# waldstein94/Stratified-Transformer

Measured on AMD Instinct MI355X. Metric: points/sec through StratifiedAttention fwd+bwd, 100k-pt scene, higher is better.
Workload: dtype f32

## Files before the change

include/pointops2_hip.h:

```cpp
#ifndef POINTOPS2_HIP_H
#define POINTOPS2_HIP_H

#include <stddef.h>
#include <stdint.h>

#ifdef __cplusplus
extern "C" {
#endif

void pointops2_set_stream(void *hip_stream);
void *pointops2_get_stream(void);
const char *pointops2_last_error(void);
int pointops2_abi_version(void);
void pointops2_diag_set_fps_patience(unsigned long long ticks_100mhz);


void furthestsampling_cuda_launcher(int b, int n, const float *xyz, const int *offset,
                                    const int *new_offset, float *tmp, int *idx);

void knnquery_cuda_launcher(int m, int nsample, const float *xyz, const float *new_xyz,
                            const int *offset, const int *new_offset, int *idx, float *dist2);

void grouping_forward_cuda_launcher(int m, int nsample, int c, const float *input, const int *idx, float *output);
void grouping_backward_cuda_launcher(int m, int nsample, int c, const float *grad_output, const int *idx, float *grad_input);
// ... 164 lines not shown
size_t pointops2_cell_plan_workspace_bytes(int N);
void pointops2_cell_plan_count_launcher(int N, int max_queries, const int *s_cluster, const int *s_starts, const int *l_cluster,
                                        const int *ls_starts, int *cell_order, int *qcell, int *cell_desc, int *cell_qstart,
                                        int *cell_kbase, int *cell_pbase, int *cell_perm, int *parent_first, int *counts, void *ws,
                                        size_t ws_bytes);
void pointops2_cell_plan_prepare_launcher(int N, int max_queries, const int *s_cluster, const int *l_cluster, int *cell_order,
                                          int *parent_first, int *counts, void *ws, size_t ws_bytes);
void pointops2_cell_plan_sizes_launcher(int N, const int *s_cluster, const int *s_starts, const int *l_cluster, const int *ls_starts,
                                        const int *cell_order, int *qcell, int *cell_desc, int *cell_qstart, int *cell_kbase,
                                        int *cell_pbase, int *cell_perm, int *counts, void *ws, size_t ws_bytes);
void pointops2_cell_plan_fill_launcher(int N, const float *xyz, float window, float quant, int L, const int *s_order, const int *ls,
                                       const float *wc, const int *cell_order, const int *qcell, const int *cell_qstart,
                                       const int *cell_desc, const int *cell_kbase, const int *cell_pbase, int *cell_keys, int *kcell,
                                       unsigned int *relp);
void pointops2_swin_quant_launcher(int N, const float *xyz, const float *bbox6, float window, float quant, int shifted, int *q);
void pointops2_swin_pairs_rel_launcher(int N, int M, const int *index_0, const int *index_1, const int *q, int qgl, int *rel_idx);
void pointops2_swin_cell_fill_launcher(int N, int L, int qgl, const int *q, const int *s_order, const int *ls, const float *wc,
                                       const int *cell_order, const int *qcell, const int *cell_qstart, const int *cell_desc,
                                       const int *cell_kbase, const int *cell_pbase, int *cell_keys, int *kcell, unsigned int *relp);
void cell_attention_forward_launcher(const pointops2_cell_plan *plan, int h, int hdim, int L, const float *q, const float *k,
                                     const float *v, const float *table_q, const float *table_k, const float *table_v, float *out,
                                     float *ml, float *pbuf);
void cell_attention_backward_launcher(const pointops2_cell_plan *plan, int h, int hdim, int L, const float *grad_out, const float *q,
                                      const float *k, const float *v, const float *out, const float *table_q, const float *table_k,
                                      const float *table_v, const float *pbuf, float *gsbuf, float *grad_q, float *grad_k,
                                      float *grad_v, float *grad_table_q, float *grad_table_k, float *grad_table_v);
#define POINTOPS2_CELL_FWD_ERROR   (-1)
#define POINTOPS2_CELL_FWD_NONE    0
#define POINTOPS2_CELL_FWD_MFMA64  1
#define POINTOPS2_CELL_FWD_MFMA80  2
#define POINTOPS2_CELL_FWD_VALU80  3
#define POINTOPS2_CELL_FWD_VALU160 4
int pointops2_cell_forward_variant(const pointops2_cell_plan *plan, int h, int hdim, int L, int bf16);

void pointops2_voxel_keys_launcher(int N, int is_f64, const void *coord, double voxel, unsigned long long *keys);
void pointops2_crop_dist_launcher(int N, int is_f64, const void *coord, int seed, void *dist);

void cell_attention_forward_bf16_launcher(const pointops2_cell_plan *plan, int h, int hdim, int L, const uint16_t *q, const uint16_t *k,
                                          const uint16_t *v, const uint16_t *table_q, const uint16_t *table_k, const uint16_t *table_v,
                                          float *out, float *ml, float *pbuf);
void cell_attention_backward_bf16_launcher(const pointops2_cell_plan *plan, int h, int hdim, int L, const float *grad_out, const uint16_t *q,
                                           const uint16_t *k, const uint16_t *v, const float *out, const uint16_t *table_q,
                                           const uint16_t *table_k, const uint16_t *table_v, const float *pbuf, float *gsbuf, float *grad_q,
                                           float *grad_k, float *grad_v, float *grad_table_q, float *grad_table_k, float *grad_table_v);
#define POINTOPS2_ROWS_F32  0
#define POINTOPS2_ROWS_F16  1
#define POINTOPS2_ROWS_BF16 2
void cell_attention_qkv_forward_launcher(const pointops2_cell_plan *plan, int h, int hdim, int L, const void *qkv, int row_type, float scale,
                                         const float *table_q, const float *table_k, const float *table_v, float *out, float *ml, float *pbuf);
void cell_attention_qkv_backward_launcher(const pointops2_cell_plan *plan, int h, int hdim, int L, const float *grad_out, const void *qkv, int row_type,
                                          float scale, const float *out, const float *table_q, const float *table_k, const float *table_v,
                                          const float *pbuf, float *gsbuf, float *grad_qkv, float *grad_table_q, float *grad_table_k,
                                          float *grad_table_v);

void kpconv_aggregate_forward_launcher(int n_q, int n_s, int n_nb, int c, int n_kp, const float *query_xyz, const float *support_xyz,
                                       const int *neighbors, const float *feat, const float *k_points, float extent, float *wf);
void kpconv_aggregate_backward_launcher(int n_q, int n_s, int n_nb, int c, int n_kp, const float *query_xyz, const float *support_xyz,
                                        const int *neighbors, const float *k_points, float extent, const float *grad_wf,
                                        float *grad_feat);

void grouped_max_forward_launcher(int m, int n_s, int k, int c, int row_type, const void *feat, const int *idx, void *out,
                                  unsigned char *arg);
void grouped_max_backward_launcher(int m, int n_s, int k, int c, int row_type, const void *grad_out, const unsigned char *arg,
                                   const int *src_offsets, const int *src_pair, void *grad_feat);

void residual_norm_forward_launcher(int n, int c, int y_type, int o_type, const float *x, const void *y, const float *s, const float *gamma,
// ... 124 lines not shown
```

stratified_transformer_amd/_lib.py:

```python
import ctypes
import os
import subprocess

import torch

_HERE = os.path.dirname(os.path.abspath(__file__))
LIB_PATH = os.path.join(_HERE, "lib", "libpointops2_hip.so")
CSRC = os.path.join(_HERE, "csrc")
_lib = None

I, U, P, Z, F, D = ctypes.c_int, ctypes.c_uint, ctypes.c_void_p, ctypes.c_size_t, ctypes.c_float, ctypes.c_double
Q = ctypes.c_longlong


class LaunchOpts(ctypes.Structure):
    _fields_ = [("table_rows", I), ("key_rows", I), ("csc_offsets", P), ("csc_pair", P), ("csc_query", P), ("row_order", P),
                ("row_order_rows", I), ("workspace", P), ("workspace_bytes", Z), ("point_count", I), ("batch_count", I),
                ("fps_prev_idx", P), ("fps_prev_new_offset", P), ("fps_unordered", I)]


def with_table_rows(opts, L):
    opts = opts if opts is not None else LaunchOpts()
    opts.table_rows = int(L)
    return opts
# ... 80 lines not shown
    "pointops2_dbscan_core_launcher": [I, I, P, P, P, P, P, P, P, P],
    "pointops2_dbscan_round_launcher": [I, I, P, P, P, P, P, P, P],
    "pointops2_dbscan_label_launcher": [I, I, P, P, P, P, P, P, P, P],
    "pointops2_contacts_count_launcher": [I, I, P, P, P, F, P, P],
    "pointops2_contacts_min_launcher": [I, I, P, P],
    "pointops2_label_boxes_launcher": [I, I, P, P, P, P, P],
    "pointops2_reach_rows_launcher": [I, I, P, P, P, F, P],
    "pointops2_supports_keys_launcher": [I, I, P, P, P, D, I, I, I, P],
    "pointops2_supports_means_launcher": [I, I, I, P, P, P, P, P, P, P, P],
    "pointops2_supports_count_launcher": [I, P, P, F, I, P],
    "pointops2_evaltile_seed_dist_launcher": [I, I, P, P, P, P, P, P],
    "pointops2_evaltile_update_launcher": [I, I, I, P, P, P, P, P],
    "pointops2_evaltile_vote_launcher": [I, I, I, I, P, P, P, P, P],
    "pointops2_evaltile_vote_shift_launcher": [I, I, I, I, P, I, P, P, P, P, P, P],
    "pointops2_augment_pass_launcher": [I] * 6 + [P] * 10,
    "pointops2_augment_blur_launcher": [Q, I, I, P, P, P],
    "optim_adamw_step_launcher": [I, I, P, P, Z, P, P, I],
    "optim_step_launcher": [I, I, I, P, P, Z, P, P, I, D, P],
    "residual_norm_stream_forward_launcher": [I, I, I, I, I, P, P, P, P, P, F, P, P, P],
    "residual_norm_stream_backward_launcher": [I, I, I, I, I, P, P, P, P, P, P, P, P, P, I, P, P],
}
RESULTS = {
    "pointops2_get_stream": ([], P),
    "pointops2_last_error": ([], ctypes.c_char_p),
    "pointops2_abi_version": ([], I),
    "pointops2_csc_workspace_bytes": ([I, I], Z),
    "pointops2_fps_workspace_bytes": ([I, I], Z),
    "pointops2_knn_workspace_bytes": ([I, I, I], Z),
    "pointops2_index_workspace_bytes": ([I], Z),
    "pointops2_partitions4_workspace_bytes": ([I], Z),
    "pointops2_row_order_workspace_bytes": ([I], Z),
    "pointops2_cell_plan_workspace_bytes": ([I], Z),
    "pointops2_cell_forward_variant": ([P, I, I, I, I], I),
    "pointops2_evaltile_max_parts": ([], I),
    "pointops2_optim_workspace_bytes": ([I, I], Z),
    "pointops2_optim_step_workspace_bytes": ([I, I, Q], Z),
}
OPTIM_KINDS = {"adamw": 0, "sgd": 1}

CELL_FWD = {"error": -1, "none": 0, "mfma64": 1, "mfma80": 2, "valu80": 3, "valu160": 4}
ROW_TYPES = {torch.float32: 0, torch.float16: 1, torch.bfloat16: 2}
ACTIVATIONS = {"none": 0, "relu": 1, "leaky_relu": 2, "tanh": 3}


def cell_forward_variant(plan, h, L, bf16=False, hdim=16):
    arg = None if plan is None else plan.c_arg() if hasattr(plan, "c_arg") else ctypes.byref(plan)
    code = lib().pointops2_cell_forward_variant(arg, int(h), int(hdim), int(L), int(bool(bf16)))
    return {v: k for k, v in CELL_FWD.items()}[code]


def exported_symbols():
    return sorted(list(SIGNATURES) + list(RESULTS))


def build(verbose=False):
    cmd = ["make", "-C", CSRC, "-j8"] + ([] if verbose else ["-s"])
    subprocess.check_call(cmd)
    return LIB_PATH


def lib():
    global _lib
    if _lib is None:
        if not os.path.exists(LIB_PATH):
            raise RuntimeError(
                f"{LIB_PATH} is missing: the HIP extension has not been built "
                "(run `python -c 'import __graft_entry__ as g; g.build()'` or `make -C stratified_transformer_amd/csrc`). "
                "There is no CPU fallback for the product path.")
        l = ctypes.CDLL(LIB_PATH)
        for name, argtypes in SIGNATURES.items():
            fn = getattr(l, name)
            fn.argtypes = argtypes
            fn.restype = None
        for name, (argtypes, restype) in RESULTS.items():
            fn = getattr(l, name)
            fn.argtypes = argtypes
            fn.restype = restype
        _lib = l
    return _lib


# ... 37 lines not shown
```

stratified_transformer_amd/csrc/cell_attn.hip:

```cpp
#include "cell_common.h"

namespace p2 {


template <typename T>
__device__ __forceinline__ void stage_table_t(T *lds, const T *__restrict__ tab, int L, int h, int head) {
    const int total = 3 * L * 16;
    for (int x = threadIdx.x; x < total; x += blockDim.x) {
        const int i = x % 16, r = (x / 16) % L, ax = x / (16 * L);
        lds[x] = tab[(((size_t)r * h + head) * 16 + i) * 3 + ax];
    }
}
template <int TS, typename T>
__device__ __forceinline__ void stage_tables(T *lds, const T *__restrict__ table_q, const T *__restrict__ table_k, const T *__restrict__ table_v, int L,
                                             int h, int head) {
    stage_table_t<T>(lds, table_q, L, h, head);
    stage_table_t<T>(lds + TS, table_k, L, h, head);
    stage_table_t<T>(lds + 2 * TS, table_v, L, h, head);
    __syncthreads();
}

template <int LCAP>
struct TabGeo {
    static constexpr int TS = 3 * LCAP * 16;
// ... 68 lines not shown
    __device__ __forceinline__ float4 q_row4(const RT *q, int i) const {
        if constexpr (PK) return scaled_row4<RT>(q + (size_t)i * rs_packed + hoff, qscale);
        else return ld_row4(q + (size_t)i * C + hoff);
    }
};
template <typename TT, bool PK>
__device__ __forceinline__ LaneCtx<TT, PK> make_lane_ctx(const TT *lds, int h, int L, int rs, float qscale) {
    LaneCtx<TT, PK> x;
    x.lds = lds;
    x.L = L;
    x.h = h;
    x.head = blockIdx.y;
    x.C = h * 16;
    x.rs_packed = rs;
    x.qscale = qscale;
    x.lane = threadIdx.x & 63;
    x.p = x.lane >> 2;
    x.c = x.lane & 3;
    x.hoff = x.head * 16 + 4 * x.c;
    return x;
}

__device__ __forceinline__ void wait_vmem() {
    asm volatile("" ::: "memory");
    __builtin_amdgcn_s_waitcnt(0x0F70);
}
__device__ __forceinline__ int next_query_ids(rsrc_t qid, int off) {
    const int ids = (int)bload_u32(qid, off);
    wait_vmem();
    return ids;
}

template <int NPA, typename RT, typename T, bool PK>
__device__ __forceinline__ void load_key_rows(const LaneCtx<T, PK> &x, const CellBufs &cb, const RT *__restrict__ rows, int j0, int nvalid,
                                              float4 (&r4)[NPA]) {
    unsigned keys[NPA];
    bload_words<NPA>(cb.key, (j0 + x.p * NPA) * 4, keys);
#pragma unroll
    for (int t = 0; t < NPA; t++) {
        const float4 r = ld_row4(rows + (size_t)keys[t] * x.rs() + x.hoff);
        r4[t] = t < nvalid ? r : make_float4(0.f, 0.f, 0.f, 0.f);
    }
}

template <int NPA, int TS, typename RT, typename T, bool PK>
__device__ __forceinline__ void fwd_sweep_logits(const LaneCtx<T, PK> &x, const CellTask &ct, const CellBufs &cb, rsrc_t rs_p,
                                                 const RT *__restrict__ q, const RT *__restrict__ k, float *__restrict__ ml,
                                                 int ch, bool single, int j0, int nkc) {
    const int p = x.p, c = x.c;
    const int nvalid = min(max(nkc - p * NPA, 0), NPA);
    float4 k4[NPA];
    load_key_rows<NPA, RT, T, PK>(x, cb, k, j0, nvalid, k4);
    int ids = (int)bload_u32(cb.qid, x.lane * 4);
    int i_nx = __builtin_amdgcn_readlane(ids, 0);
    float4 q4_nx = x.q_row4(q, i_nx);
    unsigned w_nx[NPA];
    bload_words<NPA>(cb.rel, (j0 + p * NPA) * 4, w_nx);
    float lg_pv[NPA];
#pragma unroll
    for (int t = 0; t < NPA; t++) lg_pv[t] = 0.f;
#pragma unroll 1
    for (int il = 0; il < ct.nq; il++) {
        wait_vmem();
        const int i = i_nx;
        const float4 q4 = q4_nx;
        unsigned w[NPA];
#pragma unroll
        for (int t = 0; t < NPA; t++) w[t] = w_nx[t];
        const int roff = (il * ct.nk + j0 + p * NPA) * 4;
        if (((il + 1) & 63) == 0) ids = next_query_ids(cb.qid, (il + 1 + x.lane) * 4);
        i_nx = __builtin_amdgcn_readlane(ids, (il + 1) & 63);
        q4_nx = x.q_row4(q, i_nx);
        bload_words<NPA>(cb.rel, roff + ct.nk * 4, w_nx);
        if (single && il && c == 0) bstore_floats<NPA>(rs_p, roff - ct.nk * 4, lg_pv, nvalid);
        float lg[NPA];
// ... 111 lines not shown
                                                                 const T *__restrict__ table_v, float *__restrict__ out,
                                                                 float *__restrict__ ml, float *__restrict__ pbuf, size_t plane) {
    constexpr int TS = TabGeo<LCAP>::TS;
    extern __shared__ float lds_raw[];
    T *lds = reinterpret_cast<T *>(lds_raw);
    const LaneCtx<T, PK> x = make_lane_ctx<T, PK>(lds, h, L, rs, qscale);
    const int wave = __builtin_amdgcn_readfirstlane(threadIdx.x >> 6);
    stage_tables<TS, T>(lds, table_q, table_k, table_v, L, h, x.head);
    const int nC = share_count(pl, pl.counts[0]);
    float *pb = pbuf + (size_t)x.head * plane;
    const int slots = gridDim.x * CA_WAVES, slot = blockIdx.x * CA_WAVES + wave;
    for (int round = 0; round * slots < nC; round++) {
        const int task = snake_task(round, slot, slots);
        if (task >= nC) continue;
        const CellTask ct = cell_task(pl, share_task(pl, task));
        const int nch = (ct.nk + 16 * NP - 1) / (16 * NP);
        const CellBufs cb = make_cell_bufs(pl, ct);
        const rsrc_t rs_p = tile_rsrc(pb, ct);
        for (int ch = 0; ch < nch; ch++) {
            const int j0 = ch * 16 * NP, nkc = min(16 * NP, ct.nk - j0);
            dispatch_passes<NP>((nkc + 15) >> 4, [&](auto tag) {
                fwd_sweep_logits<decltype(tag)::value, TS, RT, T, PK>(x, ct, cb, rs_p, q, k, ml, ch, nch == 1, j0, nkc);
            });
        }
        for (int ch = 0; ch < nch; ch++) {
            const int j0 = ch * 16 * NP, nkc = min(16 * NP, ct.nk - j0);
            dispatch_passes<NP>((nkc + 15) >> 4, [&](auto tag) {
                fwd_sweep_values<decltype(tag)::value, TS, RT, T, PK>(x, ct, cb, rs_p, v, ml, out, ch, nch == 1, j0, nkc);
            });
        }
    }
}

template <int NPA, typename T, bool PK>
__device__ __forceinline__ void flush_key_grads(float *scr, const float4 (&acc)[NPA], rsrc_t rs_key, int j0, int nkc, float *__restrict__ grad,
                                                const LaneCtx<T, PK> &x) {
    unsigned keys[4][NPA];
#pragma unroll
    for (int kk = 0; kk < 4; kk++) bload_words<NPA>(rs_key, (j0 + ((x.lane >> 4) + 4 * kk) * NPA) * 4, keys[kk]);
    wait_vmem();
#pragma unroll
    for (int t = 0; t < NPA; t++) {
        *reinterpret_cast<float4 *>(scr + x.p * 16 + 4 * x.c) = acc[t];
        __builtin_amdgcn_s_waitcnt(0xC07F);
        __builtin_amdgcn_wave_barrier();
#pragma unroll
        for (int kk = 0; kk < 4; kk++) {
            const int s = (x.lane >> 4) + 4 * kk;
            if (s * NPA + t < nkc) unsafeAtomicAdd(grad + (size_t)keys[kk][t] * x.rs() + x.head * 16 + (x.lane & 15), scr[s * 16 + (x.lane & 15)]);
        }
        __builtin_amdgcn_s_waitcnt(0xC07F);
        __builtin_amdgcn_wave_barrier();
    }
}

template <int NPA, int TS, typename RT, typename T, bool PK>
__device__ __forceinline__ void bwd_sweep_values(const LaneCtx<T, PK> &x, const CellTask &ct, const CellBufs &cb, rsrc_t rs_p, rsrc_t rs_g,
                                                 float *scr, const float *__restrict__ go, const float *__restrict__ out,
                                                 const RT *__restrict__ v, float *__restrict__ grad_v, int j0, int nkc) {
    const int p = x.p, c = x.c;
    const int nvalid = min(max(nkc - p * NPA, 0), NPA);
    float4 v4[NPA], dv4[NPA];
    load_key_rows<NPA, RT, T, PK>(x, cb, v, j0, nvalid, v4);
#pragma unroll
    for (int t = 0; t < NPA; t++) dv4[t] = make_float4(0.f, 0.f, 0.f, 0.f);
    unsigned w_nx[NPA];
    float a_nx[NPA];
    bload_words<NPA>(cb.rel, (j0 + p * NPA) * 4, w_nx);
    bload_floats<NPA>(rs_p, (j0 + p * NPA) * 4, a_nx);
    int ids = (int)bload_u32(cb.qid, x.lane * 4);
    int i_nx = __builtin_amdgcn_readlane(ids, 0);
    float4 go_nx = ldg4(go + (size_t)i_nx * x.C + x.hoff), o_nx = ldg4(out + (size_t)i_nx * x.C + x.hoff);
    float gs_pv[NPA];
#pragma unroll
    for (int t = 0; t < NPA; t++) gs_pv[t] = 0.f;
#pragma unroll 1
    for (int il = 0; il < ct.nq; il++) {
        wait_vmem();
        const int roff = (il * ct.nk + j0 + p * NPA) * 4;
        const float4 go4 = go_nx, o4 = o_nx;
        unsigned w[NPA];
        float a[NPA];
#pragma unroll
        for (int t = 0; t < NPA; t++) {
            w[t] = w_nx[t];
            a[t] = t < nvalid ? a_nx[t] : 0.f;
        }
        if (((il + 1) & 63) == 0) ids = next_query_ids(cb.qid, (il + 1 + x.lane) * 4);
        i_nx = __builtin_amdgcn_readlane(ids, (il + 1) & 63);
        go_nx = ldg4(go + (size_t)i_nx * x.C + x.hoff);
        o_nx = ldg4(out + (size_t)i_nx * x.C + x.hoff);
        bload_words<NPA>(cb.rel, roff + ct.nk * 4, w_nx);
        bload_floats<NPA>(rs_p, roff + ct.nk * 4, a_nx);
        if (il && c == 0) bstore_floats<NPA>(rs_g, roff - ct.nk * 4, gs_pv, nvalid);
        const float delta = quad_sum(pdot4(go4, o4));
        Rows3 rv = rows_at<2 * TS, T>(x.lds, row_off(w[0], x.L, c));
#pragma unroll
        for (int t = 0; t < NPA; t++) {
            Rows3 rv1 = rv;
            if (t + 1 < NPA) rv1 = rows_at<2 * TS, T>(x.lds, row_off(w[t + 1], x.L, c));
            const float ga = quad_sum(pdot4(go4, padd4(rsum(rv), v4[t])));
            gs_pv[t] = a[t] * (ga - delta);
            dv4[t] = pfma4(a[t], go4, dv4[t]);
            rv = rv1;
            __builtin_amdgcn_sched_barrier(0);
        }
    }
    if (ct.nq > 0 && c == 0) bstore_floats<NPA>(rs_g, ((ct.nq - 1) * ct.nk + j0 + p * NPA) * 4, gs_pv, nvalid);
    flush_key_grads<NPA, T, PK>(scr, dv4, cb.key, j0, nkc, grad_v, x);
}

template <int NPA, int TS, typename RT, typename T, bool PK>
__device__ __forceinline__ void bwd_sweep_keys(const LaneCtx<T, PK> &x, const CellTask &ct, const CellBufs &cb, rsrc_t rs_g, float *scr,
                                               const RT *__restrict__ q, const RT *__restrict__ k, float *__restrict__ grad_q,
                                               float *__restrict__ grad_k, int ch, int j0, int nkc) {
    const int p = x.p, c = x.c;
    const int nvalid = min(max(nkc - p * NPA, 0), NPA);
    float4 k4[NPA], dk4[NPA];
    load_key_rows<NPA, RT, T, PK>(x, cb, k, j0, nvalid, k4);
#pragma unroll
    for (int t = 0; t < NPA; t++) dk4[t] = make_float4(0.f, 0.f, 0.f, 0.f);
    unsigned w_nx[NPA];
    float g_nx[NPA];
    bload_words<NPA>(cb.rel, (j0 + p * NPA) * 4, w_nx);
    bload_floats<NPA>(rs_g, (j0 + p * NPA) * 4, g_nx);
    int ids = (int)bload_u32(cb.qid, x.lane * 4);
    int i_nx = __builtin_amdgcn_readlane(ids, 0);
    float4 q_nx = x.q_row4(q, i_nx);
    float4 tot_pv = make_float4(0.f, 0.f, 0.f, 0.f);
    int i_pv = 0;
    auto store_dq = [&](int i, float4 tot) {
        float *o = grad_q + (size_t)i * x.rs() + x.hoff;
        stg4(o, ch ? add4(tot, ldg4(o)) : tot);
    };
#pragma unroll 1
    for (int il = 0; il < ct.nq; il++) {
        wait_vmem();
        const int i = i_nx;
        const int roff = (il * ct.nk + j0 + p * NPA) * 4;
        const float4 q4 = q_nx;
        unsigned w[NPA];
        float g[NPA];
#pragma unroll
        for (int t = 0; t < NPA; t++) {
            w[t] = w_nx[t];
            g[t] = t < nvalid ? g_nx[t] : 0.f;
        }
        if (((il + 1) & 63) == 0) ids = next_query_ids(cb.qid, (il + 1 + x.lane) * 4);
        i_nx = __builtin_amdgcn_readlane(ids, (il + 1) & 63);
        q_nx = x.q_row4(q, i_nx);
        bload_words<NPA>(cb.rel, roff + ct.nk * 4, w_nx);
        bload_floats<NPA>(rs_g, roff + ct.nk * 4, g_nx);
        if (il && p == 0) store_dq(i_pv, tot_pv);
        float4 dq = make_float4(0.f, 0.f, 0.f, 0.f);
        RowOff ro = row_off(w[0], x.L, c);
        Rows3 rq = rows_at<0, T>(x.lds, ro), rk = rows_at<TS, T>(x.lds, ro);
#pragma unroll
        for (int t = 0; t < NPA; t++) {
            Rows3 rq1 = rq, rk1 = rk;
            if (t + 1 < NPA) {
                ro = row_off(w[t + 1], x.L, c);
                rq1 = rows_at<0, T>(x.lds, ro);
                rk1 = rows_at<TS, T>(x.lds, ro);
            }
            dq = pfma4(g[t], padd4(rsum(rq), k4[t]), dq);
            dk4[t] = pfma4(g[t], padd4(rsum(rk), q4), dk4[t]);
            rq = rq1;
            rk = rk1;
            __builtin_amdgcn_sched_barrier(0);
        }
        float4 tot = slots_sum16_4(dq);
        if constexpr (PK) tot = make_float4(tot.x * x.qscale, tot.y * x.qscale, tot.z * x.qscale, tot.w * x.qscale);
        tot_pv = tot;
        i_pv = i;
    }
    if (ct.nq > 0 && p == 0) store_dq(i_pv, tot_pv);
    flush_key_grads<NPA, T, PK>(scr, dk4, cb.key, j0, nkc, grad_k, x);
}

template <int NP, int LCAP, typename RT, typename T, bool PK>
__global__ __launch_bounds__(CA_WAVES_BWD * 64) void cell_bwd_kernel(pointops2_cell_plan pl, int h, int L, const float *__restrict__ go,
                                                                 const RT *__restrict__ q, const RT *__restrict__ k,
                                                                 const RT *__restrict__ v, int rs, float qscale, const float *__restrict__ out,
                                                                 const T *__restrict__ table_q, const T *__restrict__ table_k,
                                                                 const T *__restrict__ table_v, const float *__restrict__ pbuf,
                                                                 float *__restrict__ gsbuf, size_t plane, float *__restrict__ grad_q,
                                                                 float *__restrict__ grad_k, float *__restrict__ grad_v) {
    constexpr int TS = TabGeo<LCAP>::TS;
    extern __shared__ float lds_raw[];
    T *lds = reinterpret_cast<T *>(lds_raw);
    const LaneCtx<T, PK> x = make_lane_ctx<T, PK>(lds, h, L, rs, qscale);
    const int wave = __builtin_amdgcn_readfirstlane(threadIdx.x >> 6);
    float *scr = reinterpret_cast<float *>(lds + 3 * TS) + wave * 256;
    stage_tables<TS, T>(lds, table_q, table_k, table_v, L, h, x.head);
    const int nC = share_count(pl, pl.counts[0]);
    const float *pb = pbuf + (size_t)x.head * plane;
    float *gb = gsbuf + (size_t)x.head * plane;
    const int slots = gridDim.x * CA_WAVES_BWD, slot = blockIdx.x * CA_WAVES_BWD + wave;
    for (int round = 0; round * slots < nC; round++) {
        const int task = snake_task(round, slot, slots);
        if (task >= nC) continue;
        const CellTask ct = cell_task(pl, share_task(pl, task));
        const int nch = (ct.nk + 16 * NP - 1) / (16 * NP);
        const CellBufs cb = make_cell_bufs(pl, ct);
        const rsrc_t rs_p = tile_rsrc(pb, ct), rs_g = tile_rsrc(gb, ct);
        for (int ch = 0; ch < nch; ch++) {
            const int j0 = ch * 16 * NP, nkc = min(16 * NP, ct.nk - j0);
            dispatch_passes<NP>((nkc + 15) >> 4, [&](auto tag) {
                bwd_sweep_values<decltype(tag)::value, TS, RT, T, PK>(x, ct, cb, rs_p, rs_g, scr, go, out, v, grad_v, j0, nkc);
            });
        }
        for (int ch = 0; ch < nch; ch++) {
            const int j0 = ch * 16 * NP, nkc = min(16 * NP, ct.nk - j0);
            dispatch_passes<NP>((nkc + 15) >> 4, [&](auto tag) {
                bwd_sweep_keys<decltype(tag)::value, TS, RT, T, PK>(x, ct, cb, rs_g, scr, q, k, grad_q, grad_k, ch, j0, nkc);
            });
        }
    }
}

struct CFixScale {
    float mul, inv;
};
__device__ __forceinline__ CFixScale c_row_scale(unsigned maxbits, int n) {
    CFixScale sc;
    if (maxbits >= 0x7f800000u) {
        sc.mul = 0.f;
        sc.inv = __uint_as_float(0x7fc00000u);
        return sc;
    }
    const int E = (int)(maxbits >> 23) - 126;
    const int bits_n = 32 - __clz(max(n, 1));
    const int S = max(-126, min(126, 30 - bits_n - E));
    sc.mul = __uint_as_float((unsigned)(S + 127) << 23);
    sc.inv = __uint_as_float((unsigned)(127 - S) << 23);
    return sc;
}

constexpr int CT_WAVES = 8;

template <int TA>
struct CellTableGeo {
    static constexpr int LP = TA * 16;
    static constexpr int ROW = 3 * LP + 16;
    static constexpr size_t walk_bytes() { return (size_t)CT_WAVES * 4 * ROW * 4; }
    static constexpr size_t sum_bytes() { return (size_t)LP * 48 * 4; }
    static constexpr size_t lds_bytes() { return walk_bytes() > sum_bytes() ? walk_bytes() : sum_bytes(); }
};
// ... 177 lines not shown
static void launch_valu_fwd(hipStream_t st, const pointops2_cell_plan *plan, int h, int L, const CellRows<RT> &r, const CellTables<TT> &t, float *out, float *ml,
                            float *pbuf) {
    const size_t lds = TabGeo<LCAP>::bytes(sizeof(TT));
    allow_big_lds(cell_fwd_kernel<CA_NP, LCAP, RT, TT, PK>, lds);
    const dim3 grid(cell_grid_x(1, plan->n_cells, h, CA_WAVES), h);
    hipLaunchKernelGGL((cell_fwd_kernel<CA_NP, LCAP, RT, TT, PK>), grid, dim3(CA_WAVES * 64), lds, st, *plan, h, L, r.q, r.k, r.v, r.rs, r.scale, t.q, t.k, t.v, out,
                       ml, pbuf, (size_t)plan->n_pairs);
}

template <typename RT, typename TT, bool PK>
static void launch_cell_fwd(hipStream_t st, const pointops2_cell_plan *plan, int h, int hdim, int L, const CellRows<RT> &r, const CellTables<TT> &t, float *out,
                            float *ml, float *pbuf) {
    const char *why;
    const int variant = cell_fwd_variant(plan, h, hdim, L, !std::is_same<TT, float>::value, &why);
    if (why != nullptr) { set_error(why); return; }
    if (variant == POINTOPS2_CELL_FWD_NONE) return;
    if constexpr (std::is_same<TT, float>::value) {
        if (variant == POINTOPS2_CELL_FWD_MFMA64 || variant == POINTOPS2_CELL_FWD_MFMA80) {
            cell_fwd_mfma_launch(st, variant, plan, h, L, RowTag<RT>::code, PK, CellRows<void>{r.q, r.k, r.v, r.rs, r.scale}, t, out, pbuf);
            check_launch();
            return;
        }
    }
    if (variant == POINTOPS2_CELL_FWD_VALU80) launch_valu_fwd<80, RT, TT, PK>(st, plan, h, L, r, t, out, ml, pbuf);
    else launch_valu_fwd<160, RT, TT, PK>(st, plan, h, L, r, t, out, ml, pbuf);
    check_launch();
}

template <typename RT, typename TT, bool PK>
static void launch_cell_bwd(hipStream_t st, const pointops2_cell_plan *plan, int h, int hdim, int L, const float *grad_out, const CellRows<RT> &r, const float *out,
                            const CellTables<TT> &t, const float *pbuf, float *gsbuf, const CellGrads &g, const CellGrads &gt) {
    if (plan == nullptr || plan->n_points <= 0) return;
    if (const char *why = cell_refusal(plan, hdim, L, true)) { set_error(why); return; }
    const size_t lds = TabGeo<80>::bytes(sizeof(TT)) + (size_t)CA_WAVES_BWD * 256 * sizeof(float);
    allow_big_lds(cell_bwd_kernel<CA_NP_BWD, 80, RT, TT, PK>, lds);
    const size_t plane = (size_t)plan->n_pairs;
    hipLaunchKernelGGL((cell_bwd_kernel<CA_NP_BWD, 80, RT, TT, PK>), dim3(cell_grid_x(1, plan->n_cells, h, CA_WAVES_BWD), h),
                       dim3(CA_WAVES_BWD * 64), lds, st, *plan, h, L, grad_out, r.q, r.k, r.v, r.rs, r.scale, out, t.q, t.k, t.v, pbuf, gsbuf, plane, g.q, g.k, g.v);
    const dim3 grid3(cell_grid_x(1, plan->n_cells, h, CT_WAVES), h, 3), tblock(CT_WAVES * 64);
    if (L <= 64) hipLaunchKernelGGL((cell_table_grad3_kernel<4, RT, PK>), grid3, tblock, CellTableGeo<4>::lds_bytes(), st, *plan, h, L, gsbuf, pbuf, plane, r.q, r.k,
                                    grad_out, gt.q, gt.k, gt.v, r.rs, r.scale);
    else hipLaunchKernelGGL((cell_table_grad3_kernel<5, RT, PK>), grid3, tblock, CellTableGeo<5>::lds_bytes(), st, *plan, h, L, gsbuf, pbuf, plane, r.q, r.k, grad_out,
                            gt.q, gt.k, gt.v, r.rs, r.scale);
    check_launch();
}

template <typename RT>
static CellRows<RT> packed_rows(const void *qkv, int h, float scale) {
    const RT *r = static_cast<const RT *>(qkv);
    return {r, r + h * 16, r + 2 * h * 16, 3 * h * 16, scale};
}

}

using namespace p2;

extern "C" {

int pointops2_cell_forward_variant(const pointops2_cell_plan *plan, int h, int hdim, int L, int bf16) {
    const char *why;
    return cell_fwd_variant(plan, h, hdim, L, bf16 != 0, &why);
}

void cell_attention_forward_launcher(const pointops2_cell_plan *plan, int h, int hdim, int L, const float *q, const float *k,
                                     const float *v, const float *table_q, const float *table_k, const float *table_v, float *out,
                                     float *ml, float *pbuf) {
    launch_cell_fwd<float, float, false>(begin_launch().stream, plan, h, hdim, L, {q, k, v, h * 16, 1.0f}, {table_q, table_k, table_v}, out, ml, pbuf);
}
void cell_attention_backward_launcher(const pointops2_cell_plan *plan, int h, int hdim, int L, const float *grad_out, const float *q,
                                      const float *k, const float *v, const float *out, const float *table_q, const float *table_k,
                                      const float *table_v, const float *pbuf, float *gsbuf, float *grad_q, float *grad_k,
                                      float *grad_v, float *grad_table_q, float *grad_table_k, float *grad_table_v) {
    launch_cell_bwd<float, float, false>(begin_launch().stream, plan, h, hdim, L, grad_out, {q, k, v, h * 16, 1.0f}, out, {table_q, table_k, table_v}, pbuf, gsbuf,
                                         {grad_q, grad_k, grad_v}, {grad_table_q, grad_table_k, grad_table_v});
}
void cell_attention_forward_bf16_launcher(const pointops2_cell_plan *plan, int h, int hdim, int L, const uint16_t *q, const uint16_t *k,
                                          const uint16_t *v, const uint16_t *table_q, const uint16_t *table_k, const uint16_t *table_v,
                                          float *out, float *ml, float *pbuf) {
    launch_cell_fwd<bf16_t, bf16_t, false>(begin_launch().stream, plan, h, hdim, L, {q, k, v, h * 16, 1.0f}, {table_q, table_k, table_v}, out, ml, pbuf);
}
void cell_attention_backward_bf16_launcher(const pointops2_cell_plan *plan, int h, int hdim, int L, const float *grad_out, const uint16_t *q,
                                           const uint16_t *k, const uint16_t *v, const float *out, const uint16_t *table_q,
                                           const uint16_t *table_k, const uint16_t *table_v, const float *pbuf, float *gsbuf, float *grad_q,
                                           float *grad_k, float *grad_v, float *grad_table_q, float *grad_table_k, float *grad_table_v) {
    launch_cell_bwd<bf16_t, bf16_t, false>(begin_launch().stream, plan, h, hdim, L, grad_out, {q, k, v, h * 16, 1.0f}, out, {table_q, table_k, table_v}, pbuf, gsbuf,
                                           {grad_q, grad_k, grad_v}, {grad_table_q, grad_table_k, grad_table_v});
}

void cell_attention_qkv_forward_launcher(const pointops2_cell_plan *plan, int h, int hdim, int L, const void *qkv, int row_type, float scale,
                                         const float *table_q, const float *table_k, const float *table_v, float *out, float *ml, float *pbuf) {
    const hipStream_t st = begin_launch().stream;
    if (!with_row_type(row_type, [&](auto tag) {
        using RT = typename decltype(tag)::type;
        launch_cell_fwd<RT, float, true>(st, plan, h, hdim, L, packed_rows<RT>(qkv, h, scale), {table_q, table_k, table_v}, out, ml, pbuf);
    })) set_error("cell_attention_qkv: unknown row_type");
// ... 15 lines not shown
```

stratified_transformer_amd/csrc/cell_common.h:

```cpp
#pragma once
#include "rpe_common.h"
#include "row_types.h"
#include <algorithm>

namespace p2 {

typedef float __attribute__((ext_vector_type(4))) f32x4c;

constexpr int CA_NP = 8;
constexpr int CA_NP_BWD = 3;
constexpr int CA_WAVES = 12;
constexpr int CA_WAVES_BWD = 12;

template <int CTRL>
__device__ __forceinline__ float dppf(float v) {
    return __int_as_float(__builtin_amdgcn_update_dpp(0, __float_as_int(v), CTRL, 0xF, 0xF, true));
}
__device__ __forceinline__ float swap16(float v) { return __int_as_float(__builtin_amdgcn_ds_swizzle(__float_as_int(v), 0x401F)); }
__device__ __forceinline__ float quad_sum(float v) {
    v += dppf<0xB1>(v);
    v += dppf<0x4E>(v);
    return v;
}
__device__ __forceinline__ float slots_sum16(float v) {
    v += dppf<0x124>(v);
    v += dppf<0x128>(v);
    v += swap16(v);
    v += __shfl_xor(v, 32, 64);
    return v;
}
__device__ __forceinline__ float slots_max16(float v) {
    v = fmaxf(v, dppf<0x124>(v));
    v = fmaxf(v, dppf<0x128>(v));
    v = fmaxf(v, swap16(v));
    v = fmaxf(v, __shfl_xor(v, 32, 64));
    return v;
}
__device__ __forceinline__ float4 slots_sum16_4(float4 v) {
    return make_float4(slots_sum16(v.x), slots_sum16(v.y), slots_sum16(v.z), slots_sum16(v.w));
}

template <typename RT>
__device__ __forceinline__ float4 scaled_row4(const RT *p, float scale) {
    const float4 r = ld_row4(p);
    return make_float4(round_rows<RT>(r.x * scale), round_rows<RT>(r.y * scale), round_rows<RT>(r.z * scale), round_rows<RT>(r.w * scale));
// ... 126 lines not shown
```

Measured before the change: 9.011 million.

## Stage query blocks of rel/prob tiles and rows in per-wave LDS slices for attention backward

The backward value and key sweeps now process queries in blocks. Each block's rel-index and probability/gradient tile words, plus the go/out or q/grad_q rows, are fetched with wide buffer loads into a per-wave LDS slice. This replaces per-query scalar buffer loads with a software-prefetched chain. When a cell fits in one block and one chunk, the gradient scores are also kept in LDS so the key sweep can skip reloading them. The cost is an extra 8 KB of LDS per wave, which can lower occupancy, plus added wave barriers.

```diff
diff --git a/include/pointops2_hip.h b/include/pointops2_hip.h
--- a/include/pointops2_hip.h
+++ b/include/pointops2_hip.h
@@ -220,6 +220,9 @@
 #define POINTOPS2_CELL_FWD_VALU80  3
 #define POINTOPS2_CELL_FWD_VALU160 4
 int pointops2_cell_forward_variant(const pointops2_cell_plan *plan, int h, int hdim, int L, int bf16);
+int pointops2_cell_bwd_block_queries(int nkc);
+int pointops2_cell_bwd_staged_bytes(int nkc, int queries);
+int pointops2_cell_bwd_slice_bytes(void);
 
 void pointops2_voxel_keys_launcher(int N, int is_f64, const void *coord, double voxel, unsigned long long *keys);
 void pointops2_crop_dist_launcher(int N, int is_f64, const void *coord, int seed, void *dist);
diff --git a/stratified_transformer_amd/_lib.py b/stratified_transformer_amd/_lib.py
--- a/stratified_transformer_amd/_lib.py
+++ b/stratified_transformer_amd/_lib.py
@@ -136,6 +136,9 @@
     "pointops2_row_order_workspace_bytes": ([I], Z),
     "pointops2_cell_plan_workspace_bytes": ([I], Z),
     "pointops2_cell_forward_variant": ([P, I, I, I, I], I),
+    "pointops2_cell_bwd_block_queries": ([I], I),
+    "pointops2_cell_bwd_staged_bytes": ([I, I], I),
+    "pointops2_cell_bwd_slice_bytes": ([], I),
     "pointops2_evaltile_max_parts": ([], I),
     "pointops2_optim_workspace_bytes": ([I, I], Z),
     "pointops2_optim_step_workspace_bytes": ([I, I, Q], Z),
@@ -151,6 +154,18 @@
     arg = None if plan is None else plan.c_arg() if hasattr(plan, "c_arg") else ctypes.byref(plan)
     code = lib().pointops2_cell_forward_variant(arg, int(h), int(hdim), int(L), int(bool(bf16)))
     return {v: k for k, v in CELL_FWD.items()}[code]
+
+
+def cell_bwd_block_queries(nkc):
+    return int(lib().pointops2_cell_bwd_block_queries(int(nkc)))
+
+
+def cell_bwd_staged_bytes(nkc, queries):
+    return int(lib().pointops2_cell_bwd_staged_bytes(int(nkc), int(queries)))
+
+
+def cell_bwd_slice_bytes():
+    return int(lib().pointops2_cell_bwd_slice_bytes())
 
 
 def exported_symbols():
diff --git a/stratified_transformer_amd/csrc/cell_attn.hip b/stratified_transformer_amd/csrc/cell_attn.hip
--- a/stratified_transformer_amd/csrc/cell_attn.hip
+++ b/stratified_transformer_amd/csrc/cell_attn.hip
@@ -124,15 +124,20 @@
 }
 
 template <int NPA, typename RT, typename T, bool PK>
+__device__ __forceinline__ void load_key_rows(const LaneCtx<T, PK> &x, const CellBufs &cb, const RT *__restrict__ rows, int j0, int nvalid, int p,
+                                              int hoff, float4 (&r4)[NPA]) {
+    unsigned keys[NPA];
+    bload_words<NPA>(cb.key, (j0 + p * NPA) * 4, keys);
+#pragma unroll
+    for (int t = 0; t < NPA; t++) {
+        const float4 r = ld_row4(rows + (size_t)keys[t] * x.rs() + hoff);
+        r4[t] = t < nvalid ? r : make_float4(0.f, 0.f, 0.f, 0.f);
+    }
+}
+template <int NPA, typename RT, typename T, bool PK>
 __device__ __forceinline__ void load_key_rows(const LaneCtx<T, PK> &x, const CellBufs &cb, const RT *__restrict__ rows, int j0, int nvalid,
                                               float4 (&r4)[NPA]) {
-    unsigned keys[NPA];
-    bload_words<NPA>(cb.key, (j0 + x.p * NPA) * 4, keys);
-#pragma unroll
-    for (int t = 0; t < NPA; t++) {
-        const float4 r = ld_row4(rows + (size_t)keys[t] * x.rs() + x.hoff);
-        r4[t] = t < nvalid ? r : make_float4(0.f, 0.f, 0.f, 0.f);
-    }
+    load_key_rows<NPA, RT, T, PK>(x, cb, rows, j0, nvalid, x.p, x.hoff, r4);
 }
 
 template <int NPA, int TS, typename RT, typename T, bool PK>
@@ -310,149 +315,247 @@
     }
 }
 
+__device__ __forceinline__ int sweep_lane(int lane) {
+    asm volatile("" : "+v"(lane));
+    return lane;
+}
 template <int NPA, typename T, bool PK>
 __device__ __forceinline__ void flush_key_grads(float *scr, const float4 (&acc)[NPA], rsrc_t rs_key, int j0, int nkc, float *__restrict__ grad,
                                                 const LaneCtx<T, PK> &x) {
+    const int ln = sweep_lane(x.lane);
     unsigned keys[4][NPA];
 #pragma unroll
-    for (int kk = 0; kk < 4; kk++) bload_words<NPA>(rs_key, (j0 + ((x.lane >> 4) + 4 * kk) * NPA) * 4, keys[kk]);
+    for (int kk = 0; kk < 4; kk++) bload_words<NPA>(rs_key, (j0 + ((ln >> 4) + 4 * kk) * NPA) * 4, keys[kk]);
     wait_vmem();
 #pragma unroll
     for (int t = 0; t < NPA; t++) {
-        *reinterpret_cast<float4 *>(scr + x.p * 16 + 4 * x.c) = acc[t];
+        *reinterpret_cast<float4 *>(scr + (ln >> 2) * 16 + 4 * (ln & 3)) = acc[t];
         __builtin_amdgcn_s_waitcnt(0xC07F);
         __builtin_amdgcn_wave_barrier();
 #pragma unroll
         for (int kk = 0; kk < 4; kk++) {
-            const int s = (x.lane >> 4) + 4 * kk;
-            if (s * NPA + t < nkc) unsafeAtomicAdd(grad + (size_t)keys[kk][t] * x.rs() + x.head * 16 + (x.lane & 15), scr[s * 16 + (x.lane & 15)]);
+            const int s = (ln >> 4) + 4 * kk;
+            if (s * NPA + t < nkc) unsafeAtomicAdd(grad + (size_t)keys[kk][t] * x.rs() + x.head * 16 + (ln & 15), scr[s * 16 + (ln & 15)]);
         }
         __builtin_amdgcn_s_waitcnt(0xC07F);
         __builtin_amdgcn_wave_barrier();
     }
 }
 
+template <int NPA>
+struct BlkGeo {
+    static constexpr int W = 16 * NPA;
+    static constexpr int B = cell_bwd_block_queries(W);
+    static constexpr int LPR = W / 4;
+    static constexpr int NT = (B * LPR + 63) / 64;
+    static constexpr int NR = (B + 15) / 16;
+    static constexpr int WT = B * W, ROWS = 2 * B * W;
+    static_assert(cell_bwd_row_words(W) == W && B <= 64, "one query id per lane");
+    static_assert(cell_bwd_staged_bytes(W, B) <= CA_BWD_SLICE && (ROWS + 2 * B * 16) * 4 <= CA_BWD_SLICE, "LDS writes stay inside the slice");
+};
+__device__ __forceinline__ void lds_wave_sync() {
+    asm volatile("" ::: "memory");
+    __builtin_amdgcn_s_waitcnt(0xC07F);
+    __builtin_amdgcn_wave_barrier();
+    asm volatile("" ::: "memory");
+}
+template <int NPA>
+struct TileRegs {
+    u32x4c rel[BlkGeo<NPA>::NT], wt[BlkGeo<NPA>::NT];
+};
+template <int NPA>
+__device__ __forceinline__ void request_tile(TileRegs<NPA> &r, rsrc_t rs_rel, rsrc_t rs_wt, int lane, int nk, int j0, int b0, int bq) {
+    using G = BlkGeo<NPA>;
+#pragma unroll
+    for (int i = 0; i < G::NT; i++) {
+        const int kk = lane + 64 * i, ib = kk / G::LPR, seg = kk - ib * G::LPR;
+        r.rel[i] = r.wt[i] = u32x4c{0u, 0u, 0u, 0u};
+        if (ib < bq) {
+            const int off = ((b0 + ib) * nk + j0 + 4 * seg) * 4;
+            r.rel[i] = __builtin_amdgcn_raw_buffer_load_b128(rs_rel, off, 0, 0);
+            r.wt[i] = __builtin_amdgcn_raw_buffer_load_b128(rs_wt, off, 0, 0);
+        }
+    }
+}
+template <int NPA>
+__device__ __forceinline__ void store_tile(float *sl, const TileRegs<NPA> &r, int lane, int bq) {
+    using G = BlkGeo<NPA>;
+#pragma unroll
+    for (int i = 0; i < G::NT; i++) {
+        const int kk = lane + 64 * i;
+        if (kk / G::LPR < bq) {
+            *reinterpret_cast<u32x4c *>(sl + 4 * kk) = r.rel[i];
+            *reinterpret_cast<u32x4c *>(sl + G::WT + 4 * kk) = r.wt[i];
+        }
+    }
+}
+template <int NPA, typename F>
+__device__ __forceinline__ void request_rows(float4 (&r)[BlkGeo<NPA>::NR], int ids, int p, int bq, F row) {
+#pragma unroll
+    for (int i = 0; i < BlkGeo<NPA>::NR; i++) {
+        const int id = __shfl(ids, p + 16 * i, 64);
+        r[i] = make_float4(0.f, 0.f, 0.f, 0.f);
+        if (p + 16 * i < bq) r[i] = row(id);
+    }
+}
+template <int NPA>
+__device__ __forceinline__ void store_rows(float *rows, const float4 (&r)[BlkGeo<NPA>::NR], int p, int c, int bq) {
+#pragma unroll
+    for (int i = 0; i < BlkGeo<NPA>::NR; i++)
+        if (p + 16 * i < bq) *reinterpret_cast<float4 *>(rows + (p + 16 * i) * 16 + 4 * c) = r[i];
+}
+template <int NPA>
+__device__ __forceinline__ void slice_words(const float *arr, int ib, int p, float (&f)[NPA]) {
+#pragma unroll
+    for (int t = 0; t < NPA; t++) f[t] = arr[ib * BlkGeo<NPA>::W + p * NPA + t];
+}
+
 template <int NPA, int TS, typename RT, typename T, bool PK>
 __device__ __forceinline__ void bwd_sweep_values(const LaneCtx<T, PK> &x, const CellTask &ct, const CellBufs &cb, rsrc_t rs_p, rsrc_t rs_g,
-                                                 float *scr, const float *__restrict__ go, const float *__restrict__ out,
-                                                 const RT *__restrict__ v, float *__restrict__ grad_v, int j0, int nkc) {
-    const int p = x.p, c = x.c;
+                                                 float *scr, float *sl, const float *__restrict__ go, const float *__restrict__ out,
+                                                 const RT *__restrict__ v, float *__restrict__ grad_v, bool single, int j0, int nkc) {
+    using G = BlkGeo<NPA>;
+    const int sln = sweep_lane(x.lane), p = sln >> 2, c = sln & 3;
+    const int hoff = x.head * 16 + 4 * c;
     const int nvalid = min(max(nkc - p * NPA, 0), NPA);
+    const bool keep = single && ct.nq <= G::B;
+    float *const s_go = sl + G::ROWS, *const s_o = s_go + G::B * 16;
+    TileRegs<NPA> tr;
+    int ids = (int)bload_u32(cb.qid, sln * 4);
+    request_tile<NPA>(tr, cb.rel, rs_p, sln, ct.nk, j0, 0, min(G::B, ct.nq));
     float4 v4[NPA], dv4[NPA];
-    load_key_rows<NPA, RT, T, PK>(x, cb, v, j0, nvalid, v4);
+    load_key_rows<NPA, RT, T, PK>(x, cb, v, j0, nvalid, p, hoff, v4);
 #pragma unroll
     for (int t = 0; t < NPA; t++) dv4[t] = make_float4(0.f, 0.f, 0.f, 0.f);
-    unsigned w_nx[NPA];
-    float a_nx[NPA];
-    bload_words<NPA>(cb.rel, (j0 + p * NPA) * 4, w_nx);
-    bload_floats<NPA>(rs_p, (j0 + p * NPA) * 4, a_nx);
-    int ids = (int)bload_u32(cb.qid, x.lane * 4);
-    int i_nx = __builtin_amdgcn_readlane(ids, 0);
-    float4 go_nx = ldg4(go + (size_t)i_nx * x.C + x.hoff), o_nx = ldg4(out + (size_t)i_nx * x.C + x.hoff);
-    float gs_pv[NPA];
-#pragma unroll
-    for (int t = 0; t < NPA; t++) gs_pv[t] = 0.f;
 #pragma unroll 1
-    for (int il = 0; il < ct.nq; il++) {
+    for (int b0 = 0; b0 < ct.nq; b0 += G::B) {
+        const int bq = min(G::B, ct.nq - b0);
+        if (b0) {
+            ids = (int)bload_u32(cb.qid, (b0 + sln) * 4);
+            request_tile<NPA>(tr, cb.rel, rs_p, sln, ct.nk, j0, b0, bq);
+            wait_vmem();
+        }
+        lds_wave_sync();
+        store_tile<NPA>(sl, tr, sln, bq);
+        float4 rg[G::NR], ro[G::NR];
+        request_rows<NPA>(rg, ids, p, bq, [&](int i) { return ldg4(go + (size_t)i * x.C + hoff); });
+        request_rows<NPA>(ro, ids, p, bq, [&](int i) { return ldg4(out + (size_t)i * x.C + hoff); });
         wait_vmem();
-        const int roff = (il * ct.nk + j0 + p * NPA) * 4;
-        const float4 go4 = go_nx, o4 = o_nx;
-        unsigned w[NPA];
-        float a[NPA];
-#pragma unroll
-        for (int t = 0; t < NPA; t++) {
-            w[t] = w_nx[t];
-            a[t] = t < nvalid ? a_nx[t] : 0.f;
-        }
-        if (((il + 1) & 63) == 0) ids = next_query_ids(cb.qid, (il + 1 + x.lane) * 4);
-        i_nx = __builtin_amdgcn_readlane(ids, (il + 1) & 63);
-        go_nx = ldg4(go + (size_t)i_nx * x.C + x.hoff);
-        o_nx = ldg4(out + (size_t)i_nx * x.C + x.hoff);
-        bload_words<NPA>(cb.rel, roff + ct.nk * 4, w_nx);
-        bload_floats<NPA>(rs_p, roff + ct.nk * 4, a_nx);
-        if (il && c == 0) bstore_floats<NPA>(rs_g, roff - ct.nk * 4, gs_pv, nvalid);
-        const float delta = quad_sum(pdot4(go4, o4));
-        Rows3 rv = rows_at<2 * TS, T>(x.lds, row_off(w[0], x.L, c));
-#pragma unroll
-        for (int t = 0; t < NPA; t++) {
-            Rows3 rv1 = rv;
-            if (t + 1 < NPA) rv1 = rows_at<2 * TS, T>(x.lds, row_off(w[t + 1], x.L, c));
-            const float ga = quad_sum(pdot4(go4, padd4(rsum(rv), v4[t])));
-            gs_pv[t] = a[t] * (ga - delta);
-            dv4[t] = pfma4(a[t], go4, dv4[t]);
-            rv = rv1;
-            __builtin_amdgcn_sched_barrier(0);
-        }
-    }
-    if (ct.nq > 0 && c == 0) bstore_floats<NPA>(rs_g, ((ct.nq - 1) * ct.nk + j0 + p * NPA) * 4, gs_pv, nvalid);
+        store_rows<NPA>(s_go, rg, p, c, bq);
+        store_rows<NPA>(s_o, ro, p, c, bq);
+        lds_wave_sync();
+        float w_nx[NPA];
+        slice_words<NPA>(sl, 0, p, w_nx);
+#pragma unroll 1
+        for (int ib = 0; ib < bq; ib++) {
+            const int roff = ((b0 + ib) * ct.nk + j0 + p * NPA) * 4;
+            const float4 go4 = *reinterpret_cast<const float4 *>(s_go + ib * 16 + 4 * c), o4 = *reinterpret_cast<const float4 *>(s_o + ib * 16 + 4 * c);
+            unsigned w[NPA];
+            float a[NPA];
+            slice_words<NPA>(sl + G::WT, ib, p, a);
+#pragma unroll
+            for (int t = 0; t < NPA; t++) {
+                w[t] = __float_as_uint(w_nx[t]);
+                a[t] = t < nvalid ? a[t] : 0.f;
+            }
+            slice_words<NPA>(sl, min(ib + 1, bq - 1), p, w_nx);
+            const float delta = quad_sum(pdot4(go4, o4));
+            Rows3 rv = rows_at<2 * TS, T>(x.lds, row_off(w[0], x.L, c));
+            float gs[NPA];
+#pragma unroll
+            for (int t = 0; t < NPA; t++) {
+                Rows3 rv1 = rv;
+                if (t + 1 < NPA) rv1 = rows_at<2 * TS, T>(x.lds, row_off(w[t + 1], x.L, c));
+                const float ga = quad_sum(pdot4(go4, padd4(rsum(rv), v4[t])));
+                gs[t] = a[t] * (ga - delta);
+                dv4[t] = pfma4(a[t], go4, dv4[t]);
+                rv = rv1;
+                __builtin_amdgcn_sched_barrier(0);
+            }
+            if (c == 0) {
+                bstore_floats<NPA>(rs_g, roff, gs, nvalid);
+                if (keep) {
+#pragma unroll
+                    for (int t = 0; t < NPA; t++)
+                        if (t < nvalid) sl[G::WT + ib * G::W + p * NPA + t] = gs[t];
+                }
+            }
+        }
+    }
     flush_key_grads<NPA, T, PK>(scr, dv4, cb.key, j0, nkc, grad_v, x);
 }
 
 template <int NPA, int TS, typename RT, typename T, bool PK>
 __device__ __forceinline__ void bwd_sweep_keys(const LaneCtx<T, PK> &x, const CellTask &ct, const CellBufs &cb, rsrc_t rs_g, float *scr,
-                                               const RT *__restrict__ q, const RT *__restrict__ k, float *__restrict__ grad_q,
-                                               float *__restrict__ grad_k, int ch, int j0, int nkc) {
-    const int p = x.p, c = x.c;
+                                               float *sl, const RT *__restrict__ q, const RT *__restrict__ k, float *__restrict__ grad_q,
+                                               float *__restrict__ grad_k, int ch, bool single, int j0, int nkc) {
+    using G = BlkGeo<NPA>;
+    const int sln = sweep_lane(x.lane), p = sln >> 2, c = sln & 3;
+    const int hoff = x.head * 16 + 4 * c;
     const int nvalid = min(max(nkc - p * NPA, 0), NPA);
+    const bool kept = single && ct.nq <= G::B;
+    float *const s_q = sl + G::ROWS, *const s_dq = s_q + G::B * 16;
+    TileRegs<NPA> tr;
+    int ids = (int)bload_u32(cb.qid, sln * 4);
+    if (!kept) request_tile<NPA>(tr, cb.rel, rs_g, sln, ct.nk, j0, 0, min(G::B, ct.nq));
     float4 k4[NPA], dk4[NPA];
-    load_key_rows<NPA, RT, T, PK>(x, cb, k, j0, nvalid, k4);
+    load_key_rows<NPA, RT, T, PK>(x, cb, k, j0, nvalid, p, hoff, k4);
 #pragma unroll
     for (int t = 0; t < NPA; t++) dk4[t] = make_float4(0.f, 0.f, 0.f, 0.f);
-    unsigned w_nx[NPA];
-    float g_nx[NPA];
-    bload_words<NPA>(cb.rel, (j0 + p * NPA) * 4, w_nx);
-    bload_floats<NPA>(rs_g, (j0 + p * NPA) * 4, g_nx);
-    int ids = (int)bload_u32(cb.qid, x.lane * 4);
-    int i_nx = __builtin_amdgcn_readlane(ids, 0);
-    float4 q_nx = x.q_row4(q, i_nx);
-    float4 tot_pv = make_float4(0.f, 0.f, 0.f, 0.f);
-    int i_pv = 0;
-    auto store_dq = [&](int i, float4 tot) {
-        float *o = grad_q + (size_t)i * x.rs() + x.hoff;
-        stg4(o, ch ? add4(tot, ldg4(o)) : tot);
-    };
 #pragma unroll 1
-    for (int il = 0; il < ct.nq; il++) {
+    for (int b0 = 0; b0 < ct.nq; b0 += G::B) {
+        const int bq = min(G::B, ct.nq - b0);
+        if (b0) {
+            ids = (int)bload_u32(cb.qid, (b0 + sln) * 4);
+            request_tile<NPA>(tr, cb.rel, rs_g, sln, ct.nk, j0, b0, bq);
+            wait_vmem();
+        }
+        lds_wave_sync();
+        if (!kept) store_tile<NPA>(sl, tr, sln, bq);
+        float4 rq4[G::NR], rdq[G::NR];
+        request_rows<NPA>(rq4, ids, p, bq, [&](int i) { return x.q_row4(q + hoff - x.hoff, i); });
+        if (ch) request_rows<NPA>(rdq, ids, p, bq, [&](int i) { return ldg4(grad_q + (size_t)i * x.rs() + hoff); });
         wait_vmem();
-        const int i = i_nx;
-        const int roff = (il * ct.nk + j0 + p * NPA) * 4;
-        const float4 q4 = q_nx;
-        unsigned w[NPA];
-        float g[NPA];
-#pragma unroll
-        for (int t = 0; t < NPA; t++) {
-            w[t] = w_nx[t];
-            g[t] = t < nvalid ? g_nx[t] : 0.f;
-        }
-        if (((il + 1) & 63) == 0) ids = next_query_ids(cb.qid, (il + 1 + x.lane) * 4);
-        i_nx = __builtin_amdgcn_readlane(ids, (il + 1) & 63);
-        q_nx = x.q_row4(q, i_nx);
-        bload_words<NPA>(cb.rel, roff + ct.nk * 4, w_nx);
-        bload_floats<NPA>(rs_g, roff + ct.nk * 4, g_nx);
-        if (il && p == 0) store_dq(i_pv, tot_pv);
-        float4 dq = make_float4(0.f, 0.f, 0.f, 0.f);
-        RowOff ro = row_off(w[0], x.L, c);
-        Rows3 rq = rows_at<0, T>(x.lds, ro), rk = rows_at<TS, T>(x.lds, ro);
-#pragma unroll
-        for (int t = 0; t < NPA; t++) {
-            Rows3 rq1 = rq, rk1 = rk;
-            if (t + 1 < NPA) {
-                ro = row_off(w[t + 1], x.L, c);
-                rq1 = rows_at<0, T>(x.lds, ro);
-                rk1 = rows_at<TS, T>(x.lds, ro);
-            }
-            dq = pfma4(g[t], padd4(rsum(rq), k4[t]), dq);
-            dk4[t] = pfma4(g[t], padd4(rsum(rk), q4), dk4[t]);
-            rq = rq1;
-            rk = rk1;
-            __builtin_amdgcn_sched_barrier(0);
-        }
-        float4 tot = slots_sum16_4(dq);
-        if constexpr (PK) tot = make_float4(tot.x * x.qscale, tot.y * x.qscale, tot.z * x.qscale, tot.w * x.qscale);
-        tot_pv = tot;
-        i_pv = i;
-    }
-    if (ct.nq > 0 && p == 0) store_dq(i_pv, tot_pv);
+        store_rows<NPA>(s_q, rq4, p, c, bq);
+        if (ch) store_rows<NPA>(s_dq, rdq, p, c, bq);
+        lds_wave_sync();
+        float w_nx[NPA];
+        slice_words<NPA>(sl, 0, p, w_nx);
+#pragma unroll 1
+        for (int ib = 0; ib < bq; ib++) {
+            const int i = __builtin_amdgcn_readlane(ids, ib);
+            const float4 q4 = *reinterpret_cast<const float4 *>(s_q + ib * 16 + 4 * c);
+            unsigned w[NPA];
+            float g[NPA];
+            slice_words<NPA>(sl + G::WT, ib, p, g);
+#pragma unroll
+            for (int t = 0; t < NPA; t++) {
+                w[t] = __float_as_uint(w_nx[t]);
+                g[t] = t < nvalid ? g[t] : 0.f;
+            }
+            slice_words<NPA>(sl, min(ib + 1, bq - 1), p, w_nx);
+            float4 dq = make_float4(0.f, 0.f, 0.f, 0.f);
+            RowOff ro = row_off(w[0], x.L, c);
+            Rows3 rq = rows_at<0, T>(x.lds, ro), rk = rows_at<TS, T>(x.lds, ro);
+#pragma unroll
+            for (int t = 0; t < NPA; t++) {
+                Rows3 rq1 = rq, rk1 = rk;
+                if (t + 1 < NPA) {
+                    ro = row_off(w[t + 1], x.L, c);
+                    rq1 = rows_at<0, T>(x.lds, ro);
+                    rk1 = rows_at<TS, T>(x.lds, ro);
+                }
+                dq = pfma4(g[t], padd4(rsum(rq), k4[t]), dq);
+                dk4[t] = pfma4(g[t], padd4(rsum(rk), q4), dk4[t]);
+                rq = rq1;
+                rk = rk1;
+                __builtin_amdgcn_sched_barrier(0);
+            }
+            float4 tot = slots_sum16_4(dq);
+            if constexpr (PK) tot = make_float4(tot.x * x.qscale, tot.y * x.qscale, tot.z * x.qscale, tot.w * x.qscale);
+            if (p == 0) stg4(grad_q + (size_t)i * x.rs() + hoff, ch ? add4(tot, *reinterpret_cast<const float4 *>(s_dq + ib * 16 + 4 * c)) : tot);
+        }
+    }
     flush_key_grads<NPA, T, PK>(scr, dk4, cb.key, j0, nkc, grad_k, x);
 }
 
@@ -470,6 +573,7 @@
     const LaneCtx<T, PK> x = make_lane_ctx<T, PK>(lds, h, L, rs, qscale);
     const int wave = __builtin_amdgcn_readfirstlane(threadIdx.x >> 6);
     float *scr = reinterpret_cast<float *>(lds + 3 * TS) + wave * 256;
+    float *sl = reinterpret_cast<float *>(lds + 3 * TS) + CA_WAVES_BWD * 256 + wave * (CA_BWD_SLICE / 4);
     stage_tables<TS, T>(lds, table_q, table_k, table_v, L, h, x.head);
     const int nC = share_count(pl, pl.counts[0]);
     const float *pb = pbuf + (size_t)x.head * plane;
@@ -485,13 +589,15 @@
         for (int ch = 0; ch < nch; ch++) {
             const int j0 = ch * 16 * NP, nkc = min(16 * NP, ct.nk - j0);
             dispatch_passes<NP>((nkc + 15) >> 4, [&](auto tag) {
-                bwd_sweep_values<decltype(tag)::value, TS, RT, T, PK>(x, ct, cb, rs_p, rs_g, scr, go, out, v, grad_v, j0, nkc);
+                if constexpr (decltype(tag)::value <= NP)
+                    bwd_sweep_values<decltype(tag)::value, TS, RT, T, PK>(x, ct, cb, rs_p, rs_g, scr, sl, go, out, v, grad_v, nch == 1, j0, nkc);
             });
         }
         for (int ch = 0; ch < nch; ch++) {
             const int j0 = ch * 16 * NP, nkc = min(16 * NP, ct.nk - j0);
             dispatch_passes<NP>((nkc + 15) >> 4, [&](auto tag) {
-                bwd_sweep_keys<decltype(tag)::value, TS, RT, T, PK>(x, ct, cb, rs_g, scr, q, k, grad_q, grad_k, ch, j0, nkc);
+                if constexpr (decltype(tag)::value <= NP)
+                    bwd_sweep_keys<decltype(tag)::value, TS, RT, T, PK>(x, ct, cb, rs_g, scr, sl, q, k, grad_q, grad_k, ch, nch == 1, j0, nkc);
             });
         }
     }
@@ -735,7 +841,8 @@
                             const CellTables<TT> &t, const float *pbuf, float *gsbuf, const CellGrads &g, const CellGrads &gt) {
     if (plan == nullptr || plan->n_points <= 0) return;
     if (const char *why = cell_refusal(plan, hdim, L, true)) { set_error(why); return; }
-    const size_t lds = TabGeo<80>::bytes(sizeof(TT)) + (size_t)CA_WAVES_BWD * 256 * sizeof(float);
+    const size_t lds = TabGeo<80>::bytes(sizeof(TT)) + (size_t)CA_WAVES_BWD * 256 * sizeof(float) + (size_t)CA_WAVES_BWD * CA_BWD_SLICE;
+    static_assert(TabGeo<80>::bytes(sizeof(float)) + CA_WAVES_BWD * 256 * sizeof(float) + (size_t)CA_WAVES_BWD * CA_BWD_SLICE <= 163840, "LDS of a CU");
     allow_big_lds(cell_bwd_kernel<CA_NP_BWD, 80, RT, TT, PK>, lds);
     const size_t plane = (size_t)plan->n_pairs;
     hipLaunchKernelGGL((cell_bwd_kernel<CA_NP_BWD, 80, RT, TT, PK>), dim3(cell_grid_x(1, plan->n_cells, h, CA_WAVES_BWD), h),
@@ -764,6 +871,11 @@
     const char *why;
     return cell_fwd_variant(plan, h, hdim, L, bf16 != 0, &why);
 }
+int pointops2_cell_bwd_block_queries(int nkc) { return nkc >= 1 && nkc <= 16 * CA_NP_BWD ? cell_bwd_block_queries(nkc) : 0; }
+int pointops2_cell_bwd_staged_bytes(int nkc, int queries) {
+    return nkc >= 1 && nkc <= 16 * CA_NP_BWD && queries >= 0 ? cell_bwd_staged_bytes(nkc, queries) : -1;
+}
+int pointops2_cell_bwd_slice_bytes(void) { return CA_BWD_SLICE; }
 
 void cell_attention_forward_launcher(const pointops2_cell_plan *plan, int h, int hdim, int L, const float *q, const float *k,
                                      const float *v, const float *table_q, const float *table_k, const float *table_v, float *out,
diff --git a/stratified_transformer_amd/csrc/cell_common.h b/stratified_transformer_amd/csrc/cell_common.h
--- a/stratified_transformer_amd/csrc/cell_common.h
+++ b/stratified_transformer_amd/csrc/cell_common.h
@@ -11,6 +11,15 @@
 constexpr int CA_NP_BWD = 3;
 constexpr int CA_WAVES = 12;
 constexpr int CA_WAVES_BWD = 12;
+
+constexpr int CA_BWD_SLICE = 8192;
+__host__ __device__ constexpr int cell_bwd_row_words(int nkc) { return nkc <= 32 ? 32 : (nkc + 15) / 16 * 16; }
+__host__ __device__ constexpr int cell_bwd_staged_bytes(int nkc, int queries) { return queries * (2 * cell_bwd_row_words(nkc) + 2 * 16) * 4; }
+__host__ __device__ constexpr int cell_bwd_block_queries(int nkc) {
+    const int b = CA_BWD_SLICE / cell_bwd_staged_bytes(nkc, 1);
+    return b < 1 ? 1 : b;
+}
+static_assert(cell_bwd_staged_bytes(16 * CA_NP_BWD, cell_bwd_block_queries(16 * CA_NP_BWD)) <= CA_BWD_SLICE, "a slice holds at least one query");
 
 template <int CTRL>
 __device__ __forceinline__ float dppf(float v) {
```

Result: no change. 8.936 million (median of 2 runs) (-0.8%).
